# watsonyanghx/GAN_Lib_Tensorflow

Hardware: AMD Instinct MI355X
Metric: images/sec (G+D step) SNGAN-ResNet CIFAR-10 bs=64 (higher is better)
Workload: dtype bf16; 1 GPU; SNGAN ResNet CIFAR-10 32x32 bs=64 hinge: 1 G update (2x64 fakes) + 5 D updates (64 real + 64 fake) per step; global_batch=64, per_gpu_batch=64, parallelism=dp1, graphs=True, finite=True, collectives_in_graphs=False, grad_wire=fp32

## Files before the change

### gan_lib_tensorflow_amd/csrc/conv_igemm.hip

```cpp
#include "gank_common.h"
#include <stdlib.h>
#include <type_traits>

#define IG_IN_ZEROINS2X 16
#define IG_IN_STRIDE2 32
#define IG_RES_UP2X 128

struct IgemmArgs {
  const bf16* x;
  const bf16* w;
  const float* bias;
  const bf16* res;
  const bf16* mask;
  bf16* y;
  int N, H, W;
  int Hin, Win;
  int Cin, Cout, CoutPad, Kpad;
  int ks, pad, taps;
  int M;
  int flags;
  float scale;
  int nsteps;
  int tiles_m, tiles_n;
  int shw, sw;
// ... 903 lines not shown
                               a.res ? a.res + (long)m * a.Cout + ct : nullptr, a.y + (long)m * a.Cout + ct, h, otanh, nullptr);
      }
    }
    return;
  }
#pragma unroll
  for (int i = 0; i < 4; i++) {
    const int co0 = tile_n * 128 + i * 32 + 4 * h;
#pragma unroll
    for (int g = 0; g < 4; g++) {
      const int co = co0 + 8 * g;
      float v[4];
#pragma unroll
      for (int e = 0; e < 4; e++) v[e] = acc[i][4 * g + e] * a.scale;
      if (m < a.M && co < a.Cout) {
        const long o = (long)m * a.Cout + co;
        if (a.bias) {
          const f32x4 b = *reinterpret_cast<const f32x4*>(a.bias + co);
#pragma unroll
          for (int e = 0; e < 4; e++) v[e] += b[e];
        }
        if (a.mask) {
          const bf16x4 mk = *reinterpret_cast<const bf16x4*>(a.mask + o);
#pragma unroll
          for (int e = 0; e < 4; e++) v[e] = (bf2f(mk[e]) > 0.f) ? v[e] : 0.f;
        }
        if (a.res) {
          const bf16x4 rs = *reinterpret_cast<const bf16x4*>(a.res + o);
#pragma unroll
          for (int e = 0; e < 4; e++) v[e] += bf2f(rs[e]);
        }
        bf16x4 out;
#pragma unroll
        for (int e = 0; e < 4; e++) out[e] = f2bf(otanh ? tanhf(v[e]) : v[e]);
        *reinterpret_cast<bf16x4*>(a.y + o) = out;
      }
    }
  }
}

template <int KS, int CIN, bool POOL = false>
__global__ __launch_bounds__(256) void conv_narrow_in_kernel(IgemmArgs a) {
  __shared__ __attribute__((aligned(16))) char s_t[NARROW_LDS];
  narrow_in_body<KS, CIN, POOL>(a, blockIdx.x, s_t);
}
__global__ __launch_bounds__(256) void conv_narrow_in_pair_kernel(IgemmArgs a, IgemmArgs b, int blocks_a) {
  __shared__ __attribute__((aligned(16))) char s_t[NARROW_LDS];
  if ((int)blockIdx.x < blocks_a) narrow_in_body<3, 3, false>(a, blockIdx.x, s_t);
  else narrow_in_body<1, 3, true>(b, blockIdx.x - blocks_a, s_t);
}

template <int KS, int CIN, bool POOL = false>
static int launch_narrow_in(const IgemmArgs& a0, hipStream_t s) {
  IgemmArgs a = a0;
  a.tiles_m = cdiv(a.M, 128);
  a.tiles_n = a.CoutPad / 128;
  static const std::string tag = gank_format("conv_narrow_in_kernel<%d, %d%s>", KS, CIN, POOL ? ", pool" : "");
  gank_prof_tag(0, tag.c_str());
  hipLaunchKernelGGL((conv_narrow_in_kernel<KS, CIN, POOL>), dim3(a.tiles_m * a.tiles_n), dim3(256), 0, s, a);
  GANK_LAUNCH_OK("conv_narrow_in");
  return 0;
}

constexpr int PP_HALO_BYTES = 24576;
constexpr int PP_WSLOT_BYTES = 16384;
constexpr int PP_NSLOT = 6, PP_PD = 4;
constexpr int PP_WRING = 2 * PP_HALO_BYTES;
constexpr int PP_LDS_BYTES = PP_WRING + PP_NSLOT * PP_WSLOT_BYTES;

template <int N>
__device__ __forceinline__ void pp_wait_vmcnt() {
  static_assert(N == 0 || N == 4 || N == 6 || N == 7, "vmcnt value not instantiated");
  if constexpr (N == 0) asm volatile("s_waitcnt vmcnt(0)" ::: "memory");
  if constexpr (N == 4) asm volatile("s_waitcnt vmcnt(4)" ::: "memory");
  if constexpr (N == 6) asm volatile("s_waitcnt vmcnt(6)" ::: "memory");
  if constexpr (N == 7) asm volatile("s_waitcnt vmcnt(7)" ::: "memory");
}

#ifdef GANK_ACT_F16
#define GANK_MFMA16(a, b, c) __builtin_amdgcn_mfma_f32_16x16x32_f16(a, b, c, 0, 0, 0)
#else
#define GANK_MFMA16(a, b, c) __builtin_amdgcn_mfma_f32_16x16x32_bf16(a, b, c, 0, 0, 0)
#endif
template <int MODE, int PW, bool STATS = false>
__global__ __launch_bounds__(512) void conv_igemm_pp_kernel(IgemmArgs a) {
  constexpr bool PHASE = (MODE & 4) != 0;
  constexpr int NT = PHASE ? 4 : 9;
  constexpr int PHH = 256 / PW;
  constexpr int HW_ = PW + 2, HROW = HW_ * 64;
  constexpr int HPX = (PHH + 2) * HW_;
  auto pp_hswz = [](int hx) { return (hx >> 1) & 2; };
  auto pp_wswz = [](int co) { return (co >> 1) & 2; };
  static_assert(PW == 32 || PW == 16, "patch width");
  static_assert(HPX * 64 <= PP_HALO_BYTES, "halo image");
  extern __shared__ __attribute__((aligned(16))) char smem[];
  typedef __attribute__((address_space(3))) void* lds_t;
  const int tid = threadIdx.x, lane = tid & 63;
  const int wave = __builtin_amdgcn_readfirstlane(tid >> 6);
  const int wm = wave >> 2, wn = wave & 3;

  const int nwg = a.tiles_m * a.tiles_n;
  const int lid = xcd_remap(blockIdx.x, nwg);
  const int tile_n = lid % a.tiles_n;
  int tile_m = lid / a.tiles_n;
  int phase = 0;
  if constexpr (PHASE) {
    if (a.phase_inner) { phase = tile_m & 3; tile_m >>= 2; }
    else { phase = tile_m / a.tiles_pp; tile_m -= phase * a.tiles_pp; }
  }
  const int pad_h = PHASE ? 1 - (phase >> 1) : 1, pad_w = PHASE ? 1 - (phase & 1) : 1;
  const int pw = a.W / PW, ph = a.H / PHH;
  const int n = tile_m / (pw * ph), pr = tile_m - n * pw * ph;
  const int py0 = (pr / pw) * PHH, px0 = (pr % pw) * PW;

  constexpr unsigned OOB = 0x7FFFFFF0u;
  const __amdgpu_buffer_rsrc_t rs_x = __builtin_amdgcn_make_buffer_rsrc(const_cast<bf16*>(a.x), 0, a.N * a.H * a.W * a.Cin * 2, 0x00020000);
  const __amdgpu_buffer_rsrc_t rs_w = __builtin_amdgcn_make_buffer_rsrc(const_cast<bf16*>(a.w) + (PHASE ? (long)phase * a.CoutPad * a.Kpad : 0L), 0,
                                                                        a.CoutPad * a.Kpad * 2, 0x00020000);

  unsigned h_off[6];
#pragma unroll
  for (int j = 0; j < 6; j++) {
    const int q = (j * 4 + wn) * 64 + lane;
    const int hp = q >> 2, hy = hp / HW_, hx = hp - hy * HW_;
    const int iy = py0 - 1 + hy, ix = px0 - 1 + hx;
    const bool ok = hp < HPX && (unsigned)iy < (unsigned)a.H && (unsigned)ix < (unsigned)a.W;
    h_off[j] = ok ? (unsigned)((((n * a.H + iy) * a.W + ix) * a.Cin + (((q & 3) ^ pp_hswz(hx)) << 3)) * 2) : OOB;
  }
  int w_off[2];
#pragma unroll
  for (int j = 0; j < 2; j++) {
    const int q = (j * 8 + wave) * 64 + lane;
    const int co = q >> 2;
    w_off[j] = ((tile_n * 256 + co) * a.Kpad + (((q & 3) ^ pp_wswz(co)) << 3)) * 2;
  }
  constexpr int ND = PHASE ? 2 : 3;
  const int p16 = lane & 15, kc = lane >> 4;
  constexpr int RPT = PW / 16;
  int a_lane, b_lane[ND];
  a_lane = PP_WRING + (wn * 64 + p16) * 64 + ((kc ^ pp_wswz(p16)) << 4);
#pragma unroll
  for (int d = 0; d < ND; d++) {
    const int hx = p16 + d + (PHASE ? 1 - pad_w : 0);
    const int hy = wm * (PHH / 2) + (PHASE ? 1 - pad_h : 0);
    b_lane[d] = hy * HROW + hx * 64 + ((kc ^ pp_hswz(hx)) << 4);
  }

  const int nch = a.Cin >> 5;
  auto issue_w = [&](int slot_bytes, int c, int tap) {
    const int koff = (tap * a.Cin + c * 32) * 2;
#pragma unroll
    for (int j = 0; j < 2; j++)
      __builtin_amdgcn_raw_ptr_buffer_load_lds(rs_w, (lds_t)(smem + PP_WRING + slot_bytes + (j * 8 + wave) * 1024), 16, w_off[j], koff, 0, 0);
  };
  auto issue_h = [&](int buf, int c, int j0) {
#pragma unroll
    for (int j = j0; j < j0 + 3; j++)
      __builtin_amdgcn_raw_ptr_buffer_load_lds(rs_x, (lds_t)(smem + buf * PP_HALO_BYTES + (j * 4 + wn) * 1024), 16, (int)(h_off[j] + (unsigned)c * 64u), 0, 0, 0);
  };

  f32x4 acc[4][8];
#pragma unroll
  for (int i = 0; i < 4; i++)
#pragma unroll
    for (int j = 0; j < 8; j++) acc[i][j] = f32x4{0.f, 0.f, 0.f, 0.f};

  if (wm == 1) { issue_h(0, 0, 0); issue_h(0, 0, 3); }
  {
    int c = 0, t = 0;
#pragma unroll
    for (int q = 0; q < PP_PD; q++) {
      issue_w(q * PP_WSLOT_BYTES, c, t);
      if (++t == NT) { t = 0; c++; }
      if (c >= nch) { c = nch - 1; t = NT - 1; }
    }
  }
  pp_wait_vmcnt<4>();
  __builtin_amdgcn_s_barrier();

  int rslot = 0, wslot = PP_PD * PP_WSLOT_BYTES;
  for (int c = 0; c < nch; c++) {
    const int hb = (c & 1) * PP_HALO_BYTES;
    const int cn = (c + 1 < nch) ? c + 1 : nch - 1;
    auto phase_step = [&](auto tc) {
      constexpr int t = decltype(tc)::value;
      constexpr int dh1 = PHASE ? t / 2 : t / 3, dw1 = PHASE ? t % 2 : t % 3;
      if (wm == 1) __builtin_amdgcn_s_barrier();
      bf16x8 fa[4], fb[8];
#pragma unroll
      for (int i = 0; i < 4; i++) fa[i] = *reinterpret_cast<const bf16x8*>(smem + rslot + i * 1024 + a_lane);
#pragma unroll
      for (int j = 0; j < 8; j++) fb[j] = *reinterpret_cast<const bf16x8*>(smem + hb + (j / RPT + dh1) * HROW + (j % RPT) * 1024 + b_lane[dw1]);
      if constexpr (t < 2) { if (wm == 1) issue_h((c + 1) & 1, cn, 3 * t); }
      {
        constexpr int t4 = (t + PP_PD) % NT;
        int c4 = c + (t + PP_PD) / NT, tt = t4;
        if (c4 >= nch) { c4 = nch - 1; tt = NT - 1; }
        issue_w(wslot, c4, tt);
      }
      if constexpr (t < 2) { if (wm == 1) pp_wait_vmcnt<7>(); else pp_wait_vmcnt<4>(); }
      else pp_wait_vmcnt<4>();
      if (wm == 0) __builtin_amdgcn_s_barrier();
      asm volatile("s_waitcnt lgkmcnt(0)" ::: "memory");
      if constexpr ((MODE & 1) != 0) {
#pragma unroll
        for (int j = 0; j < 8; j++) fb[j] = __builtin_bit_cast(bf16x8, relu_bf16x8(__builtin_bit_cast(u32x4, fb[j])));
      }
      __builtin_amdgcn_sched_barrier(0);
#pragma unroll
      for (int i = 0; i < 4; i++)
#pragma unroll
        for (int j = 0; j < 8; j++)
          acc[i][j] = GANK_MFMA16(fa[i], fb[j], acc[i][j]);
      __builtin_amdgcn_sched_barrier(0);
      rslot += PP_WSLOT_BYTES; if (rslot == PP_NSLOT * PP_WSLOT_BYTES) rslot = 0;
      wslot += PP_WSLOT_BYTES; if (wslot == PP_NSLOT * PP_WSLOT_BYTES) wslot = 0;
    };
    phase_step(std::integral_constant<int, 0>{}); phase_step(std::integral_constant<int, 1>{});
    phase_step(std::integral_constant<int, 2>{}); phase_step(std::integral_constant<int, 3>{});
    if constexpr (!PHASE) {
      phase_step(std::integral_constant<int, 4>{}); phase_step(std::integral_constant<int, 5>{}); phase_step(std::integral_constant<int, 6>{});
      phase_step(std::integral_constant<int, 7>{}); phase_step(std::integral_constant<int, 8>{});
    }
  }
  pp_wait_vmcnt<0>();

  const bool otanh = (a.flags & GANK_OUT_TANH) != 0;
  float keep1 = 0.f, keep2 = 0.f;
  {
    float st1[STATS ? 2 : 1][8], st2[STATS ? 2 : 1][8];
    if constexpr (STATS) {
#pragma unroll
      for (int P = 0; P < 2; P++)
#pragma unroll
        for (int e = 0; e < 8; e++) { st1[P][e] = 0.f; st2[P][e] = 0.f; }
    }
#pragma unroll
    for (int j = 0; j < 8; j++) {
      const int py = py0 + wm * (PHH / 2) + j / RPT, px = px0 + (j % RPT) * 16 + p16;
      const long m = PHASE ? ((long)(n * 2 * a.H + 2 * py + (phase >> 1))) * (2 * a.W) + 2 * px + (phase & 1) : ((long)(n * a.H + py)) * a.W + px;
      const long mr = (!PHASE && (a.flags & IG_RES_UP2X)) ? ((long)(n * (a.H >> 1) + (py >> 1))) * (a.W >> 1) + (px >> 1) : m;
      bf16x8 outl[2];
#pragma unroll
      for (int P = 0; P < 2; P++) {
        const int co = tile_n * 256 + wn * 64 + (2 * P + (kc & 1)) * 16 + 8 * (kc >> 1);
        float v[8];
#pragma unroll
        for (int e = 0; e < 4; e++) {
          float lo = acc[2 * P][j][e] * a.scale, hi = acc[2 * P + 1][j][e] * a.scale;
          asm volatile("s_nop 1\n\tv_permlane16_swap_b32 %0, %1" : "+v"(lo), "+v"(hi));
          v[e] = lo;
          v[4 + e] = hi;
        }
        const long o = m * a.Cout + co;
        float bb[8] = {0.f, 0.f, 0.f, 0.f, 0.f, 0.f, 0.f, 0.f}, d[8];
        if (a.bias) {
          const f32x4 b0 = *reinterpret_cast<const f32x4*>(a.bias + co), b1 = *reinterpret_cast<const f32x4*>(a.bias + co + 4);
#pragma unroll
          for (int e = 0; e < 4; e++) { bb[e] = b0[e]; bb[4 + e] = b1[e]; }
        }
#pragma unroll
        for (int e = 0; e < 8; e++) { d[e] = v[e]; v[e] += bb[e]; }
        if (a.mask) {
          const bf16x8 mk = *reinterpret_cast<const bf16x8*>(a.mask + o);
#pragma unroll
          for (int e = 0; e < 8; e++) { const bool on = bf2f(mk[e]) > 0.f; v[e] = on ? v[e] : 0.f; d[e] = on ? d[e] : -bb[e]; }
        }
        if (a.res) {
          const bf16x8 rs = *reinterpret_cast<const bf16x8*>(a.res + mr * a.Cout + co);
#pragma unroll
          for (int e = 0; e < 8; e++) { const float t = bf2f(rs[e]); v[e] += t; d[e] += t; }
        }
        if constexpr (STATS) {
#pragma unroll
          for (int e = 0; e < 8; e++) { st1[P][e] += d[e]; st2[P][e] += d[e] * d[e]; }
        }
#pragma unroll
        for (int e = 0; e < 8; e++) outl[P][e] = f2bf(otanh ? tanhf(v[e]) : v[e]);
      }
      bf16* line = a.y + m * a.Cout + tile_n * 256 + wn * 64 + (kc & 1) * 16 + 8 * (kc >> 1);
#pragma unroll
      for (int P = 0; P < 2; P++) *reinterpret_cast<bf16x8*>(line + 32 * P) = outl[P];
    }
    if constexpr (STATS) {
#pragma unroll
      for (int P = 0; P < 2; P++)
#pragma unroll
        for (int e = 0; e < 8; e++) {
          const float s1 = pp_row_sum(st1[P][e]), s2 = pp_row_sum(st2[P][e]);
          const bool mine = p16 == P * 8 + e;
          keep1 = mine ? s1 : keep1;
          keep2 = mine ? s2 : keep2;
        }
    }
  }
  if constexpr (STATS) {
    float* dst = a.stat_sums + ((long)(n / a.stat_n_per_group) * GANK_STAT_SLOTS + (blockIdx.x % GANK_STAT_SLOTS)) * 2 * a.Cout;
    const int co = tile_n * 256 + wn * 64 + (2 * (p16 >> 3) + (kc & 1)) * 16 + 8 * (kc >> 1) + (p16 & 7);
    atomicAdd(dst + co, keep1);
    atomicAdd(dst + a.Cout + co, keep2);
  }
}

static thread_local int tl_stats_done = 0;
__global__ void ig_zero_kernel(float* __restrict__ p, int n) {
  const int i = blockIdx.x * blockDim.x + threadIdx.x;
  if (i < n) p[i] = 0.f;
}

static void stats_zero(const IgemmArgs& a, hipStream_t s);
constexpr int T128_MIN = 192;
static bool igemm_stats_ok(const IgemmArgs& a, int BM, int BN) {
  return a.stat_sums != nullptr && !(a.flags & GANK_OUT_TANH) && a.M % BM == 0 && a.Cout % BN == 0 &&
         ((long)a.stat_n_per_group * a.H * a.W) % BM == 0;
}
template <int MODE, int PW>
static int launch_pp(const IgemmArgs& a0, hipStream_t s) {
  IgemmArgs a = a0;
  const bool stats = a.stat_sums != nullptr;
  if (stats) { tl_stats_done = 1; stats_zero(a, s); }
  constexpr bool PHASE = (MODE & 4) != 0;
  const int tiles = a.N * (a.H / (256 / PW)) * (a.W / PW);
  a.tiles_pp = tiles;
  a.phase_inner = 1;
  a.tiles_m = PHASE ? 4 * tiles : tiles;
  a.tiles_n = a.Cout / 256;
  if (PHASE) { a.Kpad = 4 * a.Cin; a.Hin = a.H; a.Win = a.W; }
  auto kern = stats ? conv_igemm_pp_kernel<MODE, PW, true> : conv_igemm_pp_kernel<MODE, PW, false>;
  if (stats) { GANK_MAX_DYNAMIC_LDS((conv_igemm_pp_kernel<MODE, PW, true>), PP_LDS_BYTES, "conv_igemm_pp"); }
  else { GANK_MAX_DYNAMIC_LDS((conv_igemm_pp_kernel<MODE, PW, false>), PP_LDS_BYTES, "conv_igemm_pp"); }
  static const std::string tag = gank_format("conv_igemm_pp_kernel<%d, %d>", MODE, PW);
  gank_prof_tag(0, tag.c_str());
  hipLaunchKernelGGL(kern, dim3(a.tiles_m * a.tiles_n), dim3(512), PP_LDS_BYTES, s, a);
  GANK_LAUNCH_OK("conv_igemm_pp");
  return 0;
}
static int pp_patch_width(int H, int W) { return (W % 32 == 0 && H % 8 == 0) ? 32 : (W % 16 == 0 && H % 16 == 0) ? 16 : 0; }
static bool pp_enough_blocks(const IgemmArgs& a, int phases) {
  const int pw = pp_patch_width(a.H, a.W);
  return pw != 0 && (long)phases * a.N * (a.H / (256 / pw)) * (a.W / pw) * (a.Cout / 256) >= 224;
}
static bool pp_phase_ok(const IgemmArgs& a) {
  return a.Cout % 256 == 0 && a.Cin % 32 == 0 && pp_enough_blocks(a, 4);
}
static int launch_pp_phase(const IgemmArgs& a, hipStream_t s) {
  const bool relu = (a.flags & GANK_IN_RELU) != 0;
  if (pp_patch_width(a.H, a.W) == 32) return relu ? launch_pp<5, 32>(a, s) : launch_pp<4, 32>(a, s);
  return relu ? launch_pp<5, 16>(a, s) : launch_pp<4, 16>(a, s);
}

template <int MODE, int BN>
static int launch_patch(const IgemmArgs& a0, hipStream_t s) {
  IgemmArgs a = a0;
  a.tiles_m = a.N * (a.H / 8) * (a.W / 16);
  a.tiles_n = a.CoutPad / BN;
  const size_t lds = ((size_t)10 * HROWP + (size_t)2 * BN * LROW) * sizeof(bf16);
  auto kern = conv_igemm_patch_kernel<MODE, BN>;
  GANK_MAX_DYNAMIC_LDS(kern, (int)lds, "conv_igemm_patch");
  static const std::string tag = gank_format("conv_igemm_patch_kernel<%d, %d>", MODE, BN);
  gank_prof_tag(0, tag.c_str());
  hipLaunchKernelGGL(kern, dim3(a.tiles_m * a.tiles_n), dim3(256), lds, s, a);
  GANK_LAUNCH_OK("conv_igemm_patch");
  return 0;
}

template <int WM, int WN, int TM, int TN, bool PACKED, int PF, int MODE>
static int launch_cfg(const IgemmArgs& a0, hipStream_t s) {
  IgemmArgs a = a0;
  constexpr int BM = WM * TM * 32, BN = WN * TN * 32;
  a.tiles_m = cdiv(a.M, BM);
  a.tiles_n = a.CoutPad / BN;
  const size_t lds = (size_t)2 * (BM + BN) * LROW * sizeof(bf16);
  static const std::string tag = gank_format("conv_igemm_kernel<%d, %d, %d, %d, %s, %d, %d>", WM, WN, TM, TN, PACKED ? "true" : "false", PF, MODE);
  gank_prof_tag(0, tag.c_str());
  if constexpr (!PACKED && MODE == 0 && TN * 16 <= 32) {
    if (igemm_stats_ok(a, BM, BN)) {
      auto kern = conv_igemm_kernel<WM, WN, TM, TN, PACKED, PF, MODE, true>;
      GANK_MAX_DYNAMIC_LDS(kern, (int)lds, "conv_igemm");
      tl_stats_done = 1;
      stats_zero(a, s);
      hipLaunchKernelGGL(kern, dim3(a.tiles_m * a.tiles_n), dim3(WM * WN * 64), lds, s, a);
      GANK_LAUNCH_OK("conv_igemm");
      return 0;
    }
  }
  auto kern = conv_igemm_kernel<WM, WN, TM, TN, PACKED, PF, MODE>;
  GANK_MAX_DYNAMIC_LDS(kern, (int)lds, "conv_igemm");
  hipLaunchKernelGGL(kern, dim3(a.tiles_m * a.tiles_n), dim3(WM * WN * 64), lds, s, a);
  GANK_LAUNCH_OK("conv_igemm");
  return 0;
}

template <int WM, int WN, int TM, int TN, int PF>
static int launch_phase(const IgemmArgs& a0, hipStream_t s) {
  IgemmArgs a = a0;
  constexpr int BM = WM * TM * 32, BN = WN * TN * 32;
  a.tiles_pp = cdiv(a.M, BM);
  a.phase_inner = 1;
  a.tiles_m = 4 * a.tiles_pp;
  a.tiles_n = a.CoutPad / BN;
  const size_t lds = (size_t)2 * (BM + BN) * LROW * sizeof(bf16);
  static const std::string tag = gank_format("conv_igemm_kernel<%d, %d, %d, %d, false, %d, 4>", WM, WN, TM, TN, PF);
  gank_prof_tag(0, tag.c_str());
  if constexpr (TN * 16 <= 32) {
    if (igemm_stats_ok(a, BM, BN)) {
      auto kern = conv_igemm_kernel<WM, WN, TM, TN, false, PF, 4, true>;
      GANK_MAX_DYNAMIC_LDS(kern, (int)lds, "conv_igemm");
      tl_stats_done = 1;
      stats_zero(a, s);
      hipLaunchKernelGGL(kern, dim3(a.tiles_m * a.tiles_n), dim3(WM * WN * 64), lds, s, a);
      GANK_LAUNCH_OK("conv_igemm_phase");
      return 0;
    }
  }
  auto kern = conv_igemm_kernel<WM, WN, TM, TN, false, PF, 4>;
  GANK_MAX_DYNAMIC_LDS(kern, (int)lds, "conv_igemm");
  hipLaunchKernelGGL(kern, dim3(a.tiles_m * a.tiles_n), dim3(WM * WN * 64), lds, s, a);
  GANK_LAUNCH_OK("conv_igemm_phase");
  return 0;
}

template <int WM, int WN, int TM, int TN, int PF>
static int launch_mode(const IgemmArgs& a, hipStream_t s) {
  const int mode = ((a.flags & GANK_IN_RELU) ? 1 : 0) | ((a.flags & (GANK_IN_UPSAMPLE2X | IG_IN_ZEROINS2X)) ? 2 : 0);
  switch (mode) {
    case 0: return launch_cfg<WM, WN, TM, TN, false, PF, 0>(a, s);
    case 1: return launch_cfg<WM, WN, TM, TN, false, PF, 1>(a, s);
    case 2: return launch_cfg<WM, WN, TM, TN, false, PF, 2>(a, s);
    default: return launch_cfg<WM, WN, TM, TN, false, PF, 3>(a, s);
  }
}

int gank_igemm_dispatch(IgemmArgs a, hipStream_t s) {
  GANK_REQUIRE(a.x && a.w && a.y, "conv_igemm: null pointer");
  GANK_REQUIRE(a.N > 0 && a.H > 0 && a.W > 0 && a.Cin > 0 && a.Cout > 0, "conv_igemm: bad shape");
  GANK_REQUIRE(a.ks >= 1 && a.ks <= 7, "conv_igemm: unsupported filter size %d", a.ks);
  GANK_REQUIRE((long)a.N * a.Hin * a.Win * a.Cin < (1L << 30) && (long)a.N * a.H * a.W * a.Cout < (1L << 40), "conv_igemm: tensor too large (32-bit byte offsets)");
  a.taps = a.ks * a.ks;
  a.CoutPad = roundup(a.Cout, 32);
  a.Kpad = roundup(a.taps * a.Cin, 64);
  a.nsteps = a.Kpad / 64;
  a.M = a.N * a.H * a.W;
  a.sw = log2_or_neg(a.W);
  a.shw = log2_or_neg(a.H * a.W);
  const bool packed = (a.Cin % 64) != 0;
  const double flops = 2.0 * a.M * (double)a.Cout * a.taps * a.Cin;
  gank_prof_begin(0, flops, s, 2.0 * ((double)a.N * a.Hin * a.Win * a.Cin + (double)a.taps * a.Cin * a.Cout + (double)a.M * a.Cout +
                                      (a.res ? (double)a.M * a.Cout / ((a.flags & IG_RES_UP2X) ? 4.0 : 1.0) : 0.0) + (a.mask ? (double)a.M * a.Cout : 0.0)));
  int rc;
  const long tiles128 = (long)cdiv(a.M, 128) * (a.CoutPad / 128);
  a.korder = 0;
  const bool patch_geom = !packed && a.ks == 3 && a.pad == 1 &&
                          !(a.flags & (GANK_IN_UPSAMPLE2X | IG_IN_ZEROINS2X | IG_IN_STRIDE2)) &&
                          a.W % 16 == 0 && a.H % 8 == 0 && a.Hin == a.H && a.Win == a.W;
  const bool patch_ok = patch_geom && (a.Cout % 4) == 0 && a.CoutPad % 128 == 0;
  const bool patch32_ok = patch_geom && a.CoutPad == 32;
  const bool narrow_ok = !(a.flags & IG_RES_UP2X) && a.Cin == 3 && (a.ks == 1 || a.ks == 3) && a.pad == (a.ks - 1) / 2 && a.CoutPad % 128 == 0 && a.Cout % 4 == 0 &&
                         !(a.flags & (GANK_IN_UPSAMPLE2X | IG_IN_ZEROINS2X | IG_IN_STRIDE2)) && a.Hin == a.H && a.Win == a.W;
  const bool pp_ok = patch_geom && a.Cout % 256 == 0 && a.Kpad == a.taps * a.Cin && pp_enough_blocks(a, 1);
  if (narrow_ok) {
    rc = a.ks == 3 ? launch_narrow_in<3, 3>(a, s) : launch_narrow_in<1, 3>(a, s);
  } else if (pp_ok) {
    const bool relu = (a.flags & GANK_IN_RELU) != 0;
    if (pp_patch_width(a.H, a.W) == 32) rc = relu ? launch_pp<1, 32>(a, s) : launch_pp<0, 32>(a, s);
    else rc = relu ? launch_pp<1, 16>(a, s) : launch_pp<0, 16>(a, s);
  } else if (patch_ok) {
    rc = (a.flags & GANK_IN_RELU) ? launch_patch<1, 128>(a, s) : launch_patch<0, 128>(a, s);
  } else if (patch32_ok && few_ok(a)) {
    rc = (a.flags & GANK_IN_RELU) ? launch_few<1>(a, s) : launch_few<0>(a, s);
  } else if (patch32_ok) {
    rc = (a.flags & GANK_IN_RELU) ? launch_patch<1, 32>(a, s) : launch_patch<0, 32>(a, s);
  } else if (packed) {
    if (a.CoutPad % 64 == 0) rc = launch_cfg<2, 2, 1, 1, true, 1, 0>(a, s);
    else rc = launch_cfg<4, 1, 2, 1, true, 1, 0>(a, s);
  } else if (a.CoutPad % 128 == 0 && tiles128 >= T128_MIN) {
    rc = launch_mode<2, 2, 2, 2, 2>(a, s);
  } else if (a.CoutPad % 64 == 0) {
    rc = launch_mode<2, 2, 1, 1, 4>(a, s);
  } else {
    rc = launch_mode<4, 1, 2, 1, 2>(a, s);
  }
  gank_prof_end(0, s);
  return rc;
}

static int stats_setup(IgemmArgs& a, float* stat_sums, int groups, int N, int Cout, hipStream_t s, int flags) {
  tl_stats_done = 0;
  if (!stat_sums) return 0;
  a.stat_prezeroed = (flags & GANK_STATS_PREZEROED) != 0;
  GANK_REQUIRE(groups > 0 && N % groups == 0, "conv statistics: batch %d not divisible by %d towers", N, groups);
  a.stat_sums = stat_sums;
  a.stat_n_per_group = N / groups;
  a.stat_groups = groups;
  return 0;
}
static void stats_zero(const IgemmArgs& a, hipStream_t s) {
  if (a.stat_prezeroed) return;
  const int n = a.stat_groups * GANK_STAT_SLOTS * 2 * a.Cout;
  hipLaunchKernelGGL(ig_zero_kernel, dim3((n + 255) / 256), dim3(256), 0, s, a.stat_sums, n);
}

static int conv2d_fprop_impl(const void* x, const void* wf, const float* bias, const void* residual,
                             const void* relu_ref, void* y, int N, int H, int W, int Cin, int Cout, int ksize,
                             int flags, float scale, float* stat_sums, int groups, void* stream) {
  GANK_REQUIRE(ksize % 2 == 1, "conv2d_fprop: even filter sizes are not on this path (ksize=%d)", ksize);
  GANK_REQUIRE(!(flags & GANK_IN_UPSAMPLE2X) || (H % 2 == 0 && W % 2 == 0), "conv2d_fprop: upsample needs even output size");
  IgemmArgs a{};
  a.x = (const bf16*)x; a.w = (const bf16*)wf; a.bias = bias; a.res = (const bf16*)residual;
  a.mask = (const bf16*)relu_ref; a.y = (bf16*)y;
  a.N = N; a.H = H; a.W = W;
  const bool up = flags & GANK_IN_UPSAMPLE2X;
  a.Hin = up ? H / 2 : H; a.Win = up ? W / 2 : W;
  a.Cin = Cin; a.Cout = Cout; a.ks = ksize; a.pad = (ksize - 1) / 2;
  a.flags = (flags & (GANK_IN_UPSAMPLE2X | GANK_IN_RELU | GANK_OUT_TANH)) |
            ((flags & GANK_RES_UPSAMPLE2X) ? IG_RES_UP2X : 0);
  GANK_REQUIRE(!(flags & GANK_RES_UPSAMPLE2X) || (residual && H % 2 == 0 && W % 2 == 0), "conv2d_fprop: RES_UPSAMPLE2X needs a residual and even output size");
  a.scale = scale;
  if (stats_setup(a, stat_sums, groups, N, Cout, (hipStream_t)stream, flags)) return 1;
  return gank_igemm_dispatch(a, (hipStream_t)stream);
}

extern "C" int gank_conv2d_fprop(const void* x, const void* wf, const float* bias, const void* residual,
                                 const void* relu_ref, void* y, int N, int H, int W, int Cin, int Cout, int ksize,
                                 int flags, float scale, void* stream) {
  return conv2d_fprop_impl(x, wf, bias, residual, relu_ref, y, N, H, W, Cin, Cout, ksize, flags, scale, nullptr, 0, stream);
}
extern "C" int gank_conv2d_fprop_stats(const void* x, const void* wf, const float* bias, const void* residual,
                                       const void* relu_ref, void* y, int N, int H, int W, int Cin, int Cout, int ksize,
                                       int flags, float scale, float* stat_sums, int groups, int* produced, void* stream) {
  GANK_REQUIRE(stat_sums && produced, "conv2d_fprop_stats: null statistics pointers");
  const int rc = conv2d_fprop_impl(x, wf, bias, residual, relu_ref, y, N, H, W, Cin, Cout, ksize, flags, scale, stat_sums, groups, stream);
  *produced = tl_stats_done;
  return rc;
}

extern "C" int gank_cbn_relu_conv3x3_fprop(const void* x, const int32_t* labels, const float* gamma, const float* beta, const float* stats,
                                           const void* wf, const float* bias, void* y, int N, int H, int W, int Cin, int Cout,
                                           int groups, int n_labels, int flags, void* stream) {
  GANK_REQUIRE(x && labels && gamma && beta && stats && wf && y, "cbn_relu_conv3x3_fprop: null pointer");
  GANK_REQUIRE(groups > 0 && N % groups == 0 && n_labels > 0, "cbn_relu_conv3x3_fprop: batch %d / %d towers", N, groups);
  GANK_REQUIRE(Cin % 64 == 0 && W % 16 == 0 && H % 8 == 0, "cbn_relu_conv3x3_fprop: needs Cin %% 64 == 0, W %% 16 == 0, H %% 8 == 0");
  IgemmArgs a{};
  a.x = (const bf16*)x; a.w = (const bf16*)wf; a.bias = bias; a.y = (bf16*)y;
  a.N = N; a.H = H; a.W = W; a.Hin = H; a.Win = W; a.Cin = Cin; a.Cout = Cout; a.ks = 3; a.pad = 1;
  a.flags = flags & GANK_OUT_TANH;
  a.scale = 1.f;
  a.taps = 9; a.CoutPad = roundup(Cout, 32); a.Kpad = roundup(9 * Cin, 64); a.nsteps = a.Kpad / 64;
  a.M = N * H * W; a.sw = log2_or_neg(W); a.shw = log2_or_neg(H * W);
  GANK_REQUIRE(a.CoutPad == 32 || a.CoutPad % 128 == 0, "cbn_relu_conv3x3_fprop: Cout must pad to 32 or a multiple of 128 (got %d)", Cout);
  GANK_REQUIRE((long)N * H * W * Cin < (1L << 30), "cbn_relu_conv3x3_fprop: tensor too large (32-bit byte offsets)");
  a.cbn_stats = stats; a.cbn_gamma = gamma; a.cbn_beta = beta; a.cbn_labels = labels;
  a.cbn_n_per_group = N / groups; a.cbn_n_labels = n_labels;
  hipStream_t s = (hipStream_t)stream;
  gank_prof_begin(0, 2.0 * a.M * (double)Cout * 9 * Cin, s, 2.0 * ((double)a.M * Cin + 9.0 * Cin * Cout + (double)a.M * Cout));
  const int rc = a.CoutPad == 32 ? (few_ok(a) ? launch_few<8>(a, s) : launch_patch<8, 32>(a, s)) : launch_patch<8, 128>(a, s);
  gank_prof_end(0, s);
  return rc;
}

extern "C" int gank_meanpool_conv1x1_fprop(const void* x, const void* wf, const float* bias, void* y, void* pooled,
                                           int N, int H, int W, int Cin, int Cout, void* stream) {
  GANK_REQUIRE(x && wf && y && N > 0 && H > 0 && W > 0, "meanpool_conv1x1_fprop: bad arguments");
  GANK_REQUIRE(Cin == 3, "meanpool_conv1x1_fprop: built for 3-channel images (Cin = %d)", Cin);
  IgemmArgs a{};
  a.x = (const bf16*)x; a.w = (const bf16*)wf; a.bias = bias; a.y = (bf16*)y; a.aux_out = (bf16*)pooled;
  a.N = N; a.H = H; a.W = W; a.Hin = 2 * H; a.Win = 2 * W; a.Cin = Cin; a.Cout = Cout; a.ks = 1; a.pad = 0;
  a.scale = 1.f;
  a.taps = 1; a.CoutPad = roundup(Cout, 32); a.Kpad = roundup(Cin, 64); a.nsteps = a.Kpad / 64;
  a.M = N * H * W; a.sw = log2_or_neg(W); a.shw = log2_or_neg(H * W);
  GANK_REQUIRE(a.CoutPad % 128 == 0 && Cout % 4 == 0, "meanpool_conv1x1_fprop: Cout must be a multiple of 4 that pads to a multiple of 128 (got %d)", Cout);
  GANK_REQUIRE((long)N * 4 * H * W * Cin < (1L << 30), "meanpool_conv1x1_fprop: tensor too large (32-bit offsets)");
  hipStream_t s = (hipStream_t)stream;
  gank_prof_begin(0, 2.0 * a.M * (double)Cout * Cin, s, 2.0 * (4.0 * a.M * Cin + (double)Cin * Cout + (double)a.M * Cout));
  const int rc = launch_narrow_in<1, 3, true>(a, s);
  gank_prof_end(0, s);
  return rc;
}

extern "C" int gank_image_conv_pair_fprop(const void* x, const void* wf1, const float* bias1, void* y1, const void* wfs, const float* biass, void* ys,
                                          void* pooled, int N, int H, int W, int Cout1, int Couts, void* stream) {
  GANK_REQUIRE(x && wf1 && y1 && wfs && ys && N > 0 && H > 0 && W > 0 && H % 2 == 0 && W % 2 == 0, "image_conv_pair_fprop: bad arguments");
  GANK_REQUIRE(Cout1 % 128 == 0 && Couts % 128 == 0, "image_conv_pair_fprop: channel counts must be multiples of 128 (got %d, %d)", Cout1, Couts);
  GANK_REQUIRE((long)N * H * W * 3 < (1L << 30) && (long)N * H * W * Cout1 < (1L << 31), "image_conv_pair_fprop: tensor too large (32-bit offsets)");
  IgemmArgs a{}, b{};
  a.x = (const bf16*)x; a.w = (const bf16*)wf1; a.bias = bias1; a.y = (bf16*)y1;
  a.N = N; a.H = H; a.W = W; a.Hin = H; a.Win = W; a.Cin = 3; a.Cout = Cout1; a.ks = 3; a.pad = 1; a.scale = 1.f;
  a.taps = 9; a.CoutPad = Cout1; a.Kpad = roundup(27, 64); a.nsteps = 1;
  a.M = N * H * W; a.sw = log2_or_neg(W); a.shw = log2_or_neg(H * W);
  a.tiles_m = cdiv(a.M, 128); a.tiles_n = a.CoutPad / 128;
  a.korder = 0;
  const int Hp = H / 2, Wp = W / 2;
  b.x = (const bf16*)x; b.w = (const bf16*)wfs; b.bias = biass; b.y = (bf16*)ys; b.aux_out = (bf16*)pooled;
  b.N = N; b.H = Hp; b.W = Wp; b.Hin = H; b.Win = W; b.Cin = 3; b.Cout = Couts; b.ks = 1; b.pad = 0; b.scale = 1.f;
  b.taps = 1; b.CoutPad = Couts; b.Kpad = roundup(3, 64); b.nsteps = 1;
  b.M = N * Hp * Wp; b.sw = log2_or_neg(Wp); b.shw = log2_or_neg(Hp * Wp);
  b.tiles_m = cdiv(b.M, 128); b.tiles_n = b.CoutPad / 128;
  b.korder = 0;
  hipStream_t s = (hipStream_t)stream;
  const int blocks_a = a.tiles_m * a.tiles_n, blocks_b = b.tiles_m * b.tiles_n;
  gank_prof_begin(0, 2.0 * a.M * (double)Cout1 * 27 + 2.0 * b.M * (double)Couts * 3, s,
                  2.0 * ((double)a.M * 3 + 27.0 * Cout1 + (double)a.M * Cout1 + 3.0 * Couts + (double)b.M * Couts));
  gank_prof_tag(0, "conv_narrow_in_pair_kernel");
  hipLaunchKernelGGL(conv_narrow_in_pair_kernel, dim3(blocks_a + blocks_b), dim3(256), 0, s, a, b, blocks_a);
  gank_prof_end(0, s);
  GANK_LAUNCH_OK("image_conv_pair_fprop");
  return 0;
}

extern "C" int gank_conv2d_dgrad(const void* dy, const void* wd, const void* residual, const void* relu_ref, void* dx,
                                 int N, int H, int W, int Cin, int Cout, int ksize, int flags, float scale, void* stream) {
  GANK_REQUIRE(ksize % 2 == 1, "conv2d_dgrad: even filter sizes are not on this path (ksize=%d)", ksize);
  IgemmArgs a{};
  a.x = (const bf16*)dy; a.w = (const bf16*)wd; a.bias = nullptr; a.res = (const bf16*)residual;
  a.mask = (const bf16*)relu_ref; a.y = (bf16*)dx;
  a.N = N; a.H = H; a.W = W;
  const bool up = flags & GANK_IN_UPSAMPLE2X;
  a.Hin = up ? H / 2 : H; a.Win = up ? W / 2 : W;
  a.Cin = Cout; a.Cout = Cin; a.ks = ksize; a.pad = (ksize - 1) / 2;
  a.flags = (flags & (GANK_IN_UPSAMPLE2X | GANK_IN_RELU));
  a.scale = scale;
  return gank_igemm_dispatch(a, (hipStream_t)stream);
}


extern "C" int gank_conv2d_general_fprop(const void* x, const void* wf, const float* bias, void* y, int N, int Hin, int Win,
                                         int Hout, int Wout, int Cin, int Cout, int ksize, int stride, int pad, int flags, void* stream) {
  GANK_REQUIRE(stride == 1 || stride == 2, "conv2d_general_fprop: stride %d (1 or 2)", stride);
  GANK_REQUIRE(pad >= 0 && pad < ksize, "conv2d_general_fprop: pad %d outside [0, ksize)", pad);
  GANK_REQUIRE(!((flags & GANK_IN_UPSAMPLE2X) && stride == 2), "conv2d_general_fprop: upsampled input with stride 2");
  GANK_REQUIRE(Hin > 0 && Win > 0 && Hout > 0 && Wout > 0, "conv2d_general_fprop: bad sizes");
  IgemmArgs a{};
  a.x = (const bf16*)x; a.w = (const bf16*)wf; a.bias = bias; a.y = (bf16*)y;
  a.N = N; a.H = Hout; a.W = Wout; a.Hin = Hin; a.Win = Win;
  a.Cin = Cin; a.Cout = Cout; a.ks = ksize; a.pad = pad;
  a.flags = (flags & (GANK_IN_UPSAMPLE2X | GANK_IN_RELU | GANK_OUT_TANH)) | (stride == 2 ? IG_IN_STRIDE2 : 0);
  a.scale = 1.f;
  return gank_igemm_dispatch(a, (hipStream_t)stream);
}
extern "C" int gank_conv2d_general_dgrad(const void* dy, const void* wd, const void* relu_ref, void* dx, int N, int Hx, int Wx,
                                         int Hdy, int Wdy, int Cin, int Cout, int ksize, int pad, void* stream) {
  GANK_REQUIRE(pad >= 0 && pad < ksize, "conv2d_general_dgrad: pad %d outside [0, ksize)", pad);
  IgemmArgs a{};
  a.x = (const bf16*)dy; a.w = (const bf16*)wd; a.mask = (const bf16*)relu_ref; a.y = (bf16*)dx;
  a.N = N; a.H = Hx; a.W = Wx; a.Hin = Hdy; a.Win = Wdy;
  a.Cin = Cout; a.Cout = Cin; a.ks = ksize; a.pad = ksize - 1 - pad;
  a.scale = 1.f;
  return gank_igemm_dispatch(a, (hipStream_t)stream);
}

static int upconv3x3_fprop_impl(const void* x, const void* wph, const float* bias, const void* residual, void* y,
                                int N, int Hl, int Wl, int Cin, int Cout, int flags, float* stat_sums, int groups, void* stream) {
  GANK_REQUIRE(Cin % 64 == 0, "upconv3x3_fprop: Cin must be a multiple of 64 (got %d)", Cin);
  IgemmArgs a{};
  a.x = (const bf16*)x; a.w = (const bf16*)wph; a.bias = bias; a.res = (const bf16*)residual; a.y = (bf16*)y;
  a.N = N; a.H = Hl; a.W = Wl; a.Hin = Hl; a.Win = Wl;
  a.Cin = Cin; a.Cout = Cout; a.ks = 2; a.pad = 0;
  a.flags = flags & GANK_OUT_TANH;
  a.scale = 1.f;
  hipStream_t s = (hipStream_t)stream;
  a.taps = 4; a.CoutPad = roundup(Cout, 32); a.Kpad = 4 * Cin; a.nsteps = a.Kpad / 64;
  a.M = N * Hl * Wl; a.sw = log2_or_neg(Wl); a.shw = log2_or_neg(Hl * Wl);
  GANK_REQUIRE((long)N * Hl * Wl * Cin < (1L << 30) && (long)a.M * 4 * Cout < (1L << 31), "upconv3x3_fprop: tensor too large");
  if (stats_setup(a, stat_sums, groups, N, Cout, s, flags)) return 1;
  gank_prof_begin(0, 2.0 * a.M * 4.0 * (double)Cout * 4 * Cin, s, 2.0 * ((double)a.M * Cin + 16.0 * Cin * Cout + 4.0 * a.M * Cout + (residual ? 4.0 * a.M * Cout : 0.0)));
  int rc;
  const long tiles128 = 4L * cdiv(a.M, 128) * (a.CoutPad / 128);
  if (pp_phase_ok(a)) rc = launch_pp_phase(a, s);
  else if (patch_phase_ok(a)) rc = launch_patch_phase<4>(a, s);
  else if (a.CoutPad % 128 == 0 && tiles128 >= T128_MIN) rc = launch_phase<2, 2, 2, 2, 2>(a, s);
  else if (a.CoutPad % 64 == 0) rc = launch_phase<2, 2, 1, 1, 4>(a, s);
  else rc = launch_phase<4, 1, 2, 1, 2>(a, s);
  gank_prof_end(0, s);
  return rc;
}

extern "C" int gank_upconv3x3_fprop(const void* x, const void* wph, const float* bias, const void* residual, void* y,
                                    int N, int Hl, int Wl, int Cin, int Cout, int flags, void* stream) {
  return upconv3x3_fprop_impl(x, wph, bias, residual, y, N, Hl, Wl, Cin, Cout, flags, nullptr, 0, stream);
}
extern "C" int gank_upconv3x3_fprop_stats(const void* x, const void* wph, const float* bias, const void* residual, void* y,
                                          int N, int Hl, int Wl, int Cin, int Cout, int flags, float* stat_sums, int groups, int* produced,
                                          void* stream) {
  GANK_REQUIRE(stat_sums && produced, "upconv3x3_fprop_stats: null statistics pointers");
  const int rc = upconv3x3_fprop_impl(x, wph, bias, residual, y, N, Hl, Wl, Cin, Cout, flags, stat_sums, groups, stream);
  *produced = tl_stats_done;
  return rc;
}

extern "C" int gank_upconv3x3_dgrad(const void* dy, const void* wd4, const void* relu_ref, void* dx, int N, int Hl, int Wl,
                                    int Cin, int Cout, void* stream) {
  IgemmArgs a{};
  a.x = (const bf16*)dy; a.w = (const bf16*)wd4; a.mask = (const bf16*)relu_ref; a.y = (bf16*)dx;
  a.N = N; a.H = Hl; a.W = Wl; a.Hin = 2 * Hl; a.Win = 2 * Wl;
  a.Cin = Cout; a.Cout = Cin; a.ks = 4; a.pad = 1;
  a.flags = IG_IN_STRIDE2;
  a.scale = 1.f;
  return gank_igemm_dispatch(a, (hipStream_t)stream);
}

extern "C" int gank_convpool3x3_fprop(const void* x, const void* wp4, const float* bias, const void* residual, void* y,
                                      int N, int Hp, int Wp, int Cin, int Cout, int flags, void* stream) {
  IgemmArgs a{};
  a.x = (const bf16*)x; a.w = (const bf16*)wp4; a.bias = bias; a.res = (const bf16*)residual; a.y = (bf16*)y;
  a.N = N; a.H = Hp; a.W = Wp; a.Hin = 2 * Hp; a.Win = 2 * Wp;
  a.Cin = Cin; a.Cout = Cout; a.ks = 4; a.pad = 1;
  a.flags = IG_IN_STRIDE2 | (flags & GANK_IN_RELU);
  a.scale = 1.f;
  return gank_igemm_dispatch(a, (hipStream_t)stream);
}

extern "C" int gank_convpool3x3_dgrad(const void* dy, const void* wphd, const void* relu_ref, void* dx, int N, int Hp, int Wp,
                                      int Cin, int Cout, void* stream) {
  GANK_REQUIRE(Cout % 64 == 0, "convpool3x3_dgrad: Cout must be a multiple of 64 (got %d)", Cout);
  IgemmArgs a{};
  a.x = (const bf16*)dy; a.w = (const bf16*)wphd; a.mask = (const bf16*)relu_ref; a.y = (bf16*)dx;
  a.N = N; a.H = Hp; a.W = Wp; a.Hin = Hp; a.Win = Wp;
  a.Cin = Cout; a.Cout = Cin; a.ks = 2; a.pad = 0;
  a.flags = 0;
  a.scale = 1.f;
  hipStream_t s = (hipStream_t)stream;
  a.taps = 4; a.CoutPad = roundup(Cin, 32); a.Kpad = 4 * Cout; a.nsteps = a.Kpad / 64;
  a.M = N * Hp * Wp; a.sw = log2_or_neg(Wp); a.shw = log2_or_neg(Hp * Wp);
  GANK_REQUIRE((long)N * Hp * Wp * Cout < (1L << 30) && (long)a.M * 4 * Cin < (1L << 31), "convpool3x3_dgrad: tensor too large");
  gank_prof_begin(0, 2.0 * a.M * 4.0 * (double)Cin * 4 * Cout, s, 2.0 * ((double)a.M * Cout + 16.0 * Cin * Cout + 4.0 * a.M * Cin + (relu_ref ? 4.0 * a.M * Cin : 0.0)));
  int rc;
  const long tiles128 = 4L * cdiv(a.M, 128) * (a.CoutPad / 128);
  if (pp_phase_ok(a)) rc = launch_pp_phase(a, s);
  else if (patch_phase_ok(a)) rc = launch_patch_phase<4>(a, s);
  else if (a.CoutPad % 128 == 0 && tiles128 >= T128_MIN) rc = launch_phase<2, 2, 2, 2, 2>(a, s);
  else if (a.CoutPad % 64 == 0) rc = launch_phase<2, 2, 1, 1, 4>(a, s);
  else rc = launch_phase<4, 1, 2, 1, 2>(a, s);
  gank_prof_end(0, s);
  return rc;
}

static int deconv_pad_before(int ks) { int t = ks - 2; if (t < 0) t = 0; return t / 2; }

extern "C" int gank_deconv2d_fprop(const void* x, const void* wz, const float* bias, void* y, int N, int H, int W,
                                   int Cin, int Cout, int ksize, void* stream) {
  IgemmArgs a{};
  a.x = (const bf16*)x; a.w = (const bf16*)wz; a.bias = bias; a.y = (bf16*)y;
  a.N = N; a.H = 2 * H; a.W = 2 * W; a.Hin = H; a.Win = W;
  a.Cin = Cin; a.Cout = Cout; a.ks = ksize;
  a.pad = ksize - 1 - deconv_pad_before(ksize);
  a.flags = IG_IN_ZEROINS2X;
  a.scale = 1.f;
  return gank_igemm_dispatch(a, (hipStream_t)stream);
}

extern "C" int gank_deconv2d_dgrad(const void* dy, const void* wfz, void* dx, int N, int H, int W, int Cin, int Cout,
                                   int ksize, void* stream) {
  IgemmArgs a{};
  a.x = (const bf16*)dy; a.w = (const bf16*)wfz; a.y = (bf16*)dx;
  a.N = N; a.H = H; a.W = W; a.Hin = 2 * H; a.Win = 2 * W;
  a.Cin = Cout; a.Cout = Cin; a.ks = ksize; a.pad = deconv_pad_before(ksize);
  a.flags = IG_IN_STRIDE2;
  a.scale = 1.f;
  return gank_igemm_dispatch(a, (hipStream_t)stream);
}
```

Baseline: 62190 images/sec.

## Add dedicated low-resolution upconv kernel for 4x4 inputs with weight LDS ring

```diff
diff --git a/gan_lib_tensorflow_amd/csrc/conv_igemm.hip b/gan_lib_tensorflow_amd/csrc/conv_igemm.hip
--- a/gan_lib_tensorflow_amd/csrc/conv_igemm.hip
+++ b/gan_lib_tensorflow_amd/csrc/conv_igemm.hip
@@ -1229,6 +1229,173 @@
   }
 }
 
+constexpr int UL_XROW = 144;
+constexpr int UL_WSLOT = 4096;
+constexpr int UL_NSLOT = 4, UL_PD = 3;
+constexpr int ul_xbuf_bytes(int mt) { return (32 * mt + 1) * UL_XROW; }
+constexpr int ul_wring_off(int mt) { return (2 * ul_xbuf_bytes(mt) + 1023) / 1024 * 1024; }
+constexpr int ul_lds_bytes(int mt) { return ul_wring_off(mt) + 4 * UL_NSLOT * UL_WSLOT; }
+
+template <int HL, int MT, bool STATS>
+__global__ __launch_bounds__(256) void upconv_lowres_kernel(IgemmArgs a) {
+  constexpr int HW = HL * HL, BM = 32 * MT;
+  static_assert(BM % HW == 0 && HW % 16 == 0, "a tile is whole images; a 16-lane row stays inside one image");
+  static_assert(ul_lds_bytes(MT) <= 160 * 1024, "LDS");
+  static_assert(UL_NSLOT == UL_PD + 1 && 4 * UL_PD == 12, "ring: the slot written in step s was last read in step s - 1; vmcnt(12) below");
+  constexpr int XBUF = ul_xbuf_bytes(MT), WRING = ul_wring_off(MT), ZROW = BM * UL_XROW;
+  extern __shared__ __attribute__((aligned(16))) char smem[];
+  typedef __attribute__((address_space(3))) void* lds_t;
+  const int tid = threadIdx.x, lane = tid & 63;
+  const int phase = __builtin_amdgcn_readfirstlane(tid >> 6);
+  const int r = lane & 31, h = lane >> 5;
+  const int tile_n = blockIdx.x % a.tiles_n, tile_m = blockIdx.x / a.tiles_n;
+  const int co0 = tile_n * 32;
+  const int m0 = tile_m * BM;
+
+  const __amdgpu_buffer_rsrc_t rs_x = __builtin_amdgcn_make_buffer_rsrc(const_cast<bf16*>(a.x), 0, a.M * a.Cin * 2, 0x00020000);
+  const __amdgpu_buffer_rsrc_t rs_w = __builtin_amdgcn_make_buffer_rsrc(const_cast<bf16*>(a.w), 0, 4 * a.CoutPad * a.Kpad * 2, 0x00020000);
+
+  int x_off[MT];
+#pragma unroll
+  for (int j = 0; j < MT; j++) {
+    const int q = tid + 256 * j;
+    x_off[j] = ((m0 + (q >> 3)) * a.Cin + (q & 7) * 8) * 2;
+  }
+  u32x4 rX[MT];
+  auto load_x = [&](int c) {
+#pragma unroll
+    for (int j = 0; j < MT; j++) rX[j] = __builtin_amdgcn_raw_buffer_load_b128(rs_x, x_off[j] + c * 128, 0, 0);
+  };
+  auto store_x = [&](int buf) {
+#pragma unroll
+    for (int j = 0; j < MT; j++) {
+      const int q = tid + 256 * j;
+      *reinterpret_cast<u32x4*>(smem + buf * XBUF + (q >> 3) * UL_XROW + (q & 7) * 16) = rX[j];
+    }
+  };
+  int w_off[4];
+#pragma unroll
+  for (int j = 0; j < 4; j++) {
+    const int row = 8 * j + (lane >> 3);
+    w_off[j] = ((phase * a.CoutPad + co0 + row) * a.Kpad + (((lane & 7) ^ ((row >> 1) & 7)) << 3)) * 2;
+  }
+  char* const wring = smem + WRING + phase * (UL_NSLOT * UL_WSLOT);
+  const int nch = a.Cin >> 6, nsteps = 4 * nch;
+  auto issue_w = [&](int s) {
+    const int slot = s % UL_NSLOT;
+    const int sc = s < nsteps ? s : nsteps - 1;
+    const int koff = ((sc & 3) * a.Cin + (sc >> 2) * 64) * 2;
+#pragma unroll
+    for (int j = 0; j < 4; j++)
+      __builtin_amdgcn_raw_ptr_buffer_load_lds(rs_w, (lds_t)(wring + slot * UL_WSLOT + j * 1024), 16, w_off[j], koff, 0, 0);
+  };
+  const int a_row = r * 128, a_swz = (r >> 1) & 7;
+  int b_off[4][MT];
+  {
+    const int pa = phase >> 1, pb = phase & 1;
+#pragma unroll
+    for (int t = 0; t < 4; t++)
+#pragma unroll
+      for (int j = 0; j < MT; j++) {
+        const int p = 32 * j + r, pl = p % HW, y = pl / HL, x = pl % HL;
+        const int dy = (t >> 1) - 1 + pa, dx = (t & 1) - 1 + pb;
+        const bool ok = (unsigned)(y + dy) < (unsigned)HL && (unsigned)(x + dx) < (unsigned)HL;
+        b_off[t][j] = (ok ? (p + dy * HL + dx) * UL_XROW : ZROW) + h * 16;
+      }
+  }
+
+  f32x16 acc[MT];
+#pragma unroll
+  for (int j = 0; j < MT; j++)
+#pragma unroll
+    for (int e = 0; e < 16; e++) acc[j][e] = 0.f;
+
+#pragma unroll
+  for (int s = 0; s < UL_PD; s++) issue_w(s);
+  load_x(0);
+  if (tid < 18) *reinterpret_cast<u32x4*>(smem + (tid / 9) * XBUF + ZROW + (tid % 9) * 16) = u32x4{0u, 0u, 0u, 0u};
+  store_x(0);
+  if (nch > 1) load_x(1);
+  asm volatile("s_waitcnt lgkmcnt(0)" ::: "memory");
+  __builtin_amdgcn_s_barrier();
+
+  for (int c = 0; c < nch; c++) {
+    const char* xb = smem + (c & 1) * XBUF;
+#pragma unroll
+    for (int t = 0; t < 4; t++) {
+      const int s = 4 * c + t;
+      asm volatile("s_waitcnt lgkmcnt(0)" ::: "memory");
+      issue_w(s + UL_PD);
+      asm volatile("s_waitcnt vmcnt(12)" ::: "memory");
+      __builtin_amdgcn_sched_barrier(0);
+      const char* ws = wring + (s % UL_NSLOT) * UL_WSLOT + a_row;
+#pragma unroll
+      for (int kk = 0; kk < 4; kk++) {
+        const bf16x8 fa = *reinterpret_cast<const bf16x8*>(ws + (((2 * kk + h) ^ a_swz) << 4));
+#pragma unroll
+        for (int j = 0; j < MT; j++) {
+          const bf16x8 fb = *reinterpret_cast<const bf16x8*>(xb + b_off[t][j] + kk * 32);
+          acc[j] = GANK_MFMA32(fa, fb, acc[j]);
+        }
+      }
+      if (t == 1 && c + 1 < nch) {
+        store_x((c + 1) & 1);
+        if (c + 2 < nch) load_x(c + 2);
+      }
+    }
+    asm volatile("s_waitcnt lgkmcnt(0)" ::: "memory");
+    __builtin_amdgcn_s_barrier();
+  }
+  asm volatile("s_waitcnt vmcnt(0)" ::: "memory");
+
+  const bool otanh = (a.flags & GANK_OUT_TANH) != 0;
+  const int p16 = lane & 15;
+  float st1[STATS ? 16 : 1], st2[STATS ? 16 : 1];
+  int curg = -1;
+  auto flush = [&]() {
+    if constexpr (STATS) {
+      if (curg >= 0) {
+        float keep1 = 0.f, keep2 = 0.f;
+#pragma unroll
+        for (int i = 0; i < 16; i++) {
+          const float s1 = pp_row_sum(st1[i]), s2 = pp_row_sum(st2[i]);
+          keep1 = p16 == i ? s1 : keep1;
+          keep2 = p16 == i ? s2 : keep2;
+        }
+        float* dst = a.stat_sums + ((long)curg * GANK_STAT_SLOTS + (blockIdx.x % GANK_STAT_SLOTS)) * 2 * a.Cout;
+        const int co = co0 + 16 * (p16 >> 3) + 8 * h + (p16 & 7);
+        atomicAdd(dst + co, keep1);
+        atomicAdd(dst + a.Cout + co, keep2);
+      }
+#pragma unroll
+      for (int i = 0; i < 16; i++) { st1[i] = 0.f; st2[i] = 0.f; }
+    }
+  };
+  flush();
+#pragma unroll
+  for (int j = 0; j < MT; j++) {
+    const int ml = m0 + 32 * j + r;
+    const bool valid = ml < a.M;
+    const int n_ = ml / HW, pl = ml % HW;
+    if constexpr (STATS) {
+      const int g = valid ? n_ / a.stat_n_per_group : -1;
+      if (g != curg) { flush(); curg = g; }
+    }
+    if (!valid) continue;
+    const long m = ((long)(n_ * 2 * HL + 2 * (pl / HL) + (phase >> 1))) * (2 * HL) + 2 * (pl % HL) + (phase & 1);
+    float d[2][8];
+    epi_tile_wide<STATS>(acc[j], a.scale, a.bias ? a.bias + co0 : nullptr, nullptr, a.res ? a.res + m * a.Cout + co0 : nullptr,
+                         a.y + m * a.Cout + co0, h, otanh, d);
+    if constexpr (STATS) {
+#pragma unroll
+      for (int q = 0; q < 2; q++)
+#pragma unroll
+        for (int e = 0; e < 8; e++) { st1[q * 8 + e] += d[q][e]; st2[q * 8 + e] += d[q][e] * d[q][e]; }
+    }
+  }
+  flush();
+}
+
 static thread_local int tl_stats_done = 0;
 __global__ void ig_zero_kernel(float* __restrict__ p, int n) {
   const int i = blockIdx.x * blockDim.x + threadIdx.x;
@@ -1274,6 +1441,43 @@
   const bool relu = (a.flags & GANK_IN_RELU) != 0;
   if (pp_patch_width(a.H, a.W) == 32) return relu ? launch_pp<5, 32>(a, s) : launch_pp<4, 32>(a, s);
   return relu ? launch_pp<5, 16>(a, s) : launch_pp<4, 16>(a, s);
+}
+
+static bool upconv_lowres_ok(const IgemmArgs& a) {
+  return a.H == a.W && a.H == 4 && a.Cout % 256 == 0 && a.Cin % 64 == 0;
+}
+template <int HL, int MT>
+static int launch_upconv_lowres_cfg(const IgemmArgs& a0, hipStream_t s) {
+  IgemmArgs a = a0;
+  const bool stats = a.stat_sums != nullptr;
+  if (stats) { tl_stats_done = 1; stats_zero(a, s); }
+  a.tiles_m = cdiv(a.M, 32 * MT);
+  a.tiles_n = a.Cout / 32;
+  constexpr int lds = ul_lds_bytes(MT);
+  static const std::string tag = gank_format("upconv_lowres_kernel<%d, %d>", HL, MT);
+  gank_prof_tag(0, tag.c_str());
+  if (stats) {
+    GANK_MAX_DYNAMIC_LDS((upconv_lowres_kernel<HL, MT, true>), lds, "upconv_lowres");
+    hipLaunchKernelGGL((upconv_lowres_kernel<HL, MT, true>), dim3(a.tiles_m * a.tiles_n), dim3(256), lds, s, a);
+  } else {
+    GANK_MAX_DYNAMIC_LDS((upconv_lowres_kernel<HL, MT, false>), lds, "upconv_lowres");
+    hipLaunchKernelGGL((upconv_lowres_kernel<HL, MT, false>), dim3(a.tiles_m * a.tiles_n), dim3(256), lds, s, a);
+  }
+  GANK_LAUNCH_OK("upconv_lowres");
+  return 0;
+}
+static int launch_upconv_lowres(const IgemmArgs& a, hipStream_t s) {
+  const int hw = a.H * a.W;
+  int best = 0;
+  long best_cost = 0;
+  for (int mt : {2, 4, 5}) {
+    if ((32 * mt) % hw != 0) continue;
+    const long blocks = (long)cdiv(a.M, 32 * mt) * (a.Cout / 32);
+    const long cost = ((blocks + 255) / 256) * (16 + 3 * mt);
+    if (!best || cost < best_cost) { best = mt; best_cost = cost; }
+  }
+  if (a.H == 4) return best == 2 ? launch_upconv_lowres_cfg<4, 2>(a, s) : best == 4 ? launch_upconv_lowres_cfg<4, 4>(a, s) : launch_upconv_lowres_cfg<4, 5>(a, s);
+  return best == 2 ? launch_upconv_lowres_cfg<8, 2>(a, s) : launch_upconv_lowres_cfg<8, 4>(a, s);
 }
 
 template <int MODE, int BN>
@@ -1592,7 +1796,8 @@
   gank_prof_begin(0, 2.0 * a.M * 4.0 * (double)Cout * 4 * Cin, s, 2.0 * ((double)a.M * Cin + 16.0 * Cin * Cout + 4.0 * a.M * Cout + (residual ? 4.0 * a.M * Cout : 0.0)));
   int rc;
   const long tiles128 = 4L * cdiv(a.M, 128) * (a.CoutPad / 128);
-  if (pp_phase_ok(a)) rc = launch_pp_phase(a, s);
+  if (upconv_lowres_ok(a)) rc = launch_upconv_lowres(a, s);
+  else if (pp_phase_ok(a)) rc = launch_pp_phase(a, s);
   else if (patch_phase_ok(a)) rc = launch_patch_phase<4>(a, s);
   else if (a.CoutPad % 128 == 0 && tiles128 >= T128_MIN) rc = launch_phase<2, 2, 2, 2, 2>(a, s);
   else if (a.CoutPad % 64 == 0) rc = launch_phase<2, 2, 1, 1, 4>(a, s);
```

New measurement: 62360 images/sec, median of 3. Within noise of the previous version (+0.3%).
